# better62/MM-VQA-Healthcare

Measured on AMD Instinct MI355X. Metric: image-question pairs/sec, M3AE-base fine-tune step (fwd+bwd+AdamW) @384px, higher is better.
Workload: dtype bf16

## Files before the change

include/m3ae_hip.h:

```cpp
#ifndef M3AE_HIP_H
#define M3AE_HIP_H

#include <stdint.h>

#ifdef __cplusplus
extern "C" {
#endif

#define M3AE_ABI_VERSION 4

enum { M3AE_F32 = 0, M3AE_BF16 = 1 };
enum { M3AE_ACT_NONE = 0, M3AE_ACT_GELU = 1, M3AE_ACT_QUICKGELU = 2, M3AE_ACT_TANH = 3, M3AE_ACT_RELU = 4,
       M3AE_ACT_MULAUX = 5  };
enum { M3AE_ERR_ARG = -1, M3AE_ERR_UNSUPPORTED = -2, M3AE_ERR_ALIGN = -3, M3AE_ERR_WORKSPACE = -4 };

int m3ae_abi_version(void);
void m3ae_desc_sizes(int64_t out3[3]);
const char* m3ae_last_gemm_path(void);

typedef struct {
    int64_t M, N, K;
    int64_t batch1, batch2;
    const void* A; int64_t a_sm, a_sk, a_sb1, a_sb2;
    const void* B; int64_t b_sk, b_sn, b_sb1, b_sb2;
// ... 44 lines not shown
    float* delta;
    float* d_pos_bias;
    float dropout_p;
    uint64_t dropout_seed;
    const void* dropout_salt;
    int32_t launch_flags;
} m3ae_attn_desc;
enum { M3AE_ATTN_LEGACY_KERNELS = 1,
       M3AE_ATTN_F32_X3 = 2    };
int64_t m3ae_attn_workspace_bytes(const m3ae_attn_desc* d, int backward);
int m3ae_attn_fwd(const m3ae_attn_desc* d, void* stream);
int m3ae_attn_bwd(const m3ae_attn_desc* d, void* stream);
int m3ae_attn_fwd_rows(const m3ae_attn_desc* d, int64_t row_base, int64_t row_step, void* stream);
int m3ae_attn_bwd_rows(const m3ae_attn_desc* d, int64_t row_base, int64_t row_step, void* stream);
int m3ae_attn_probs(const m3ae_attn_desc* d, float* probs, int64_t p_sb, int64_t p_sh, int64_t p_sq, void* stream);

typedef struct {
    int32_t dir;
    int64_t B, Lq, Lk, D, H;
    const void* x;
    const void* y;
    const float* key_mask;
    const void *wq, *wq_t, *wkv, *wkv_t, *wo, *wo_t;
    const float *bq, *bkv, *bo, *ln_g, *ln_b;
    float ln_eps;
    float dropout_p;
    uint64_t seed_attn, seed_hidden;
    void* proj;
    void* prime;
    float* colbias;
// ... 147 lines not shown
```

mm-vqa-healthcare_amd/m3ae_amd/_lib.py:

```python
import ctypes as C
import os

_PKG = os.path.dirname(os.path.abspath(__file__))
DIAGNOSTIC = os.environ.get("M3AE_DIAGNOSTIC_LIB", "") == "1"
LIB_PATH = os.path.join(_PKG, "lib_diag" if DIAGNOSTIC else "lib", "libm3ae_hip.so")

F32, BF16 = 0, 1
ACT_NONE, ACT_GELU, ACT_QUICKGELU, ACT_TANH, ACT_RELU, ACT_MULAUX = 0, 1, 2, 3, 4, 5

vp, i64, i32, f32 = C.c_void_p, C.c_int64, C.c_int32, C.c_float


class GemmDesc(C.Structure):
    _fields_ = [
        ("M", i64), ("N", i64), ("K", i64), ("batch1", i64), ("batch2", i64),
        ("A", vp), ("a_sm", i64), ("a_sk", i64), ("a_sb1", i64), ("a_sb2", i64),
        ("B", vp), ("b_sk", i64), ("b_sn", i64), ("b_sb1", i64), ("b_sb2", i64),
        ("C", vp), ("c_sm", i64), ("c_sn", i64), ("c_sb1", i64), ("c_sb2", i64),
        ("dtype_a", i32), ("dtype_b", i32), ("dtype_c", i32),
        ("alpha", f32), ("accumulate", i32), ("bias", vp), ("act", i32), ("preact", vp), ("residual", vp),
        ("dact_aux", vp), ("dact", i32), ("force_generic", i32), ("a_rowsum", vp),
        ("dropout_p", f32), ("dropout_seed", C.c_uint64), ("preact_grad", i32), ("launch_flags", i32), ("dropout_salt", vp),
    ]

# ... 13 lines not shown


class XattnDesc(C.Structure):
    _fields_ = [
        ("dir", i32), ("B", i64), ("Lq", i64), ("Lk", i64), ("D", i64), ("H", i64),
        ("x", vp), ("y", vp), ("key_mask", vp),
        ("wq", vp), ("wq_t", vp), ("wkv", vp), ("wkv_t", vp), ("wo", vp), ("wo_t", vp),
        ("bq", vp), ("bkv", vp), ("bo", vp), ("ln_g", vp), ("ln_b", vp),
        ("ln_eps", f32), ("dropout_p", f32), ("seed_attn", C.c_uint64), ("seed_hidden", C.c_uint64),
        ("proj", vp), ("prime", vp), ("colbias", vp), ("probs", vp), ("probs_drop", vp), ("rowsum", vp),
        ("zctx", vp), ("ctx", vp), ("s", vp), ("out", vp), ("mean", vp), ("rstd", vp),
        ("d_out", vp), ("dx", vp), ("dy", vp),
        ("g_wq", vp), ("g_wkv", vp), ("g_wo", vp), ("g_bq", vp), ("g_bkv", vp), ("g_bo", vp), ("g_ln_g", vp), ("g_ln_b", vp),
        ("ws_ds", vp), ("ws_dsd", vp), ("ws_dscores", vp), ("ws_dprime", vp), ("ws_dproj", vp), ("ws_dz", vp), ("ws_dctx", vp),
        ("ws_vec", vp), ("ws_ln", vp), ("launch_flags", i32), ("dropout_salt", vp),
    ]


GEMM_NO_PERSISTENT, GEMM_F32_X3, GEMM_DETERMINISTIC = 1, 2, 4
DET_COLSUM, DET_EMBED_BWD, DET_BCE, DET_XENT, DET_MIM = 0, 1, 2, 3, 4
ATTN_LEGACY_KERNELS, ATTN_F32_X3 = 1, 2
XATTN_NO_PERSISTENT, XATTN_LEGACY_CHAIN = 1, 2
ABI_VERSION = 4


_SIGS = {
    "m3ae_abi_version": (C.c_int, []),
    "m3ae_desc_sizes": (None, [C.POINTER(i64)]),
    "m3ae_last_gemm_path": (C.c_char_p, []),
    "m3ae_gemm": (C.c_int, [C.POINTER(GemmDesc), vp]),
# ... 48 lines not shown
    "m3ae_xent_det": (C.c_int, [vp, vp, vp, vp, i64, i64, i64, f32, C.c_int, vp, i64, vp]),
    "m3ae_mim_loss_fwd_det": (C.c_int, [vp, vp, vp, vp, vp, i64, i64, i64, C.c_int, vp, i64, vp]),
    "m3ae_image_resample_workspace_bytes": (i64, [i64, i64]),
    "m3ae_image_resample_u8": (C.c_int, [vp, i64, vp, vp, i64, i64, i64, vp, i64, vp, vp, C.POINTER(C.c_float), C.POINTER(C.c_float), vp]),
    "m3ae_gemm_rows": (C.c_int, [C.POINTER(GemmDesc), i64, i64, vp]),
    "m3ae_attn_fwd_rows": (C.c_int, [C.POINTER(AttnDesc), i64, i64, vp]),
    "m3ae_attn_bwd_rows": (C.c_int, [C.POINTER(AttnDesc), i64, i64, vp]),
    "m3ae_layernorm_bwd_drop_rows": (C.c_int, [vp, vp, vp, vp, vp, vp, vp, vp, f32, C.c_uint64, vp, vp, vp, vp, i64, i64, C.c_int, i64, i64, vp]),
    "m3ae_dropout_rows": (C.c_int, [vp, vp, vp, i64, i64, f32, C.c_uint64, vp, C.c_int, i64, i64, vp]),
    "m3ae_beam_topk_workspace_bytes": (i64, [i64, i64, i64, i64]),
    "m3ae_beam_topk": (C.c_int, [vp, i64, vp, i64, i64, i64, i64, vp, i64, vp, vp, vp]),
    "m3ae_beam_step": (C.c_int, [vp, vp, vp, vp, vp, vp, vp, vp, vp, vp, vp, vp, vp, vp, i64, i64, i64, i64, i64, i64, i64, C.c_double, vp]),
    "m3ae_beam_finalize": (C.c_int, [vp, vp, vp, vp, vp, vp, vp, vp, vp, i64, i64, i64, i64, i64, i64, C.c_double, vp]),
    "m3ae_expand_samples": (C.c_int, [vp, vp, vp, i64, i64, i64, C.c_int, vp]),
    "m3ae_segment_sum_rows": (C.c_int, [vp, vp, vp, vp, i64, i64, i64, C.c_int, vp]),
}

EXPORTS = tuple(_SIGS)
_lib = None


class M3AEHipError(RuntimeError):
    pass


def lib():
    global _lib
    if _lib is None:
        if not os.path.exists(LIB_PATH):
            raise M3AEHipError(f"{LIB_PATH} is missing: build it with `python -m m3ae_amd.build` "
# ... 1 lines not shown
        import torch
        if DIAGNOSTIC:
            import warnings
            warnings.warn(f"m3ae_amd: loading the DIAGNOSTIC library {LIB_PATH} (timing-only builds may compute wrong results)")
        l = C.CDLL(LIB_PATH)
        for name, (res, args) in _SIGS.items():
            fn = getattr(l, name)
            fn.restype, fn.argtypes = res, args
        if l.m3ae_abi_version() != ABI_VERSION:
            raise M3AEHipError(f"ABI version mismatch: library {l.m3ae_abi_version()}, binding {ABI_VERSION}")
        sizes = (i64 * 3)()
        l.m3ae_desc_sizes(sizes)
        mine = (C.sizeof(GemmDesc), C.sizeof(AttnDesc), C.sizeof(XattnDesc))
        if tuple(sizes) != mine:
            raise M3AEHipError(f"descriptor layout mismatch: library {tuple(sizes)}, binding {mine}")
        _lib = l
    return _lib


def check(rc, what):
    if rc != 0:
        kind = {-1: "invalid argument", -2: "unsupported shape/dtype", -3: "misaligned", -4: "workspace too small"}.get(
            rc, f"hipError_t {rc}" if rc > 0 else f"error {rc}")
        raise M3AEHipError(f"{what} failed: {kind}")
```

mm-vqa-healthcare_amd/m3ae_amd/ops.py:

```python
import contextlib
import ctypes as C
import functools
import math
import os
import threading

import torch

from . import _lib
from ._lib import (ACT_GELU, ACT_MULAUX, ACT_NONE, ACT_QUICKGELU, ACT_RELU, ACT_TANH, BF16, F32, AttnDesc, GemmDesc, XattnDesc,
                   check)

grad_ready_hook = None
SAVE_DACT = os.environ.get("M3AE_SAVE_DACT", "1") != "0"
NT_NO_PERSISTENT = os.environ.get("M3AE_NT_NO_PERSISTENT", "0") == "1"
GEMM_NT_VARIANT, GEMM_TN_VARIANT, GEMM_COL_GROUP = int(os.environ.get("M3AE_GEMM_NT_VARIANT", -1)), int(os.environ.get("M3AE_GEMM_TN_VARIANT", -1)), int(os.environ.get("M3AE_GEMM_COL_GROUP", 0))


ATTN_LEGACY = os.environ.get("M3AE_ATTN_LEGACY", "0") == "1"
GEMM_ST_POLICY = int(os.environ.get("M3AE_GEMM_ST_POLICY", 0))


def _gemm_flags():
    return ((1 if NT_NO_PERSISTENT else 0) | (((GEMM_NT_VARIANT + 1) & 0xF) << 8) | (((GEMM_TN_VARIANT + 1) & 0xF) << 12)
            | ((GEMM_COL_GROUP & 0xF) << 16) | ((GEMM_ST_POLICY & 0x3) << 20))
PROFILE = None
# ... 635 lines not shown
    d = _attn_desc(B, heads, Lq, Lk, Dh, q, k, v, o, key_mask, pos_bias, scale, causal, lse, lse.shape[-1], _dt(q))
    delta = torch.empty_like(lse) if q.dtype == torch.bfloat16 else torch.zeros_like(lse)
    d.d_o, d.dq, d.dk, d.dv, d.delta = do.data_ptr(), dq.data_ptr(), dk.data_ptr(), dv.data_ptr(), delta.data_ptr()
    d.d_pos_bias = d_pos_bias.data_ptr() if d_pos_bias is not None else None
    _set_dropout(d, dropout)
    ws = _attn_ws(d, True, q.device)
    e0 = _prof_begin()
    if rows is not None:
        check(_lib.lib().m3ae_attn_bwd_rows(C.byref(d), rows[0], rows[1], _stream()), "m3ae_attn_bwd_rows")
    else:
        check(_lib.lib().m3ae_attn_bwd(C.byref(d), _stream()), "m3ae_attn_bwd")
    _prof_end(e0, "attn_bwd", (B, heads, Lq, Lk, Dh))
    del ws, delta


def attn_probs(q, k, lse, heads, key_mask=None, scale=None, dropout=None):
    _need_cuda(q)
    B, Lq, D = q.shape
    Lk = k.shape[1]
    Dh = D // heads
    if q.dtype == torch.bfloat16 and Dh != 64:
        return attn_probs(q.float(), k.float(), None, heads, key_mask, scale, dropout)
    scale = (1.0 / math.sqrt(Dh)) if scale is None else scale
    out = torch.empty((B, heads, Lq, Lk), dtype=torch.float32, device=q.device)
    lse_stride = lse.shape[-1] if lse is not None else 0
    d = _attn_desc(B, heads, Lq, Lk, Dh, q, k, k, q, key_mask, None, scale, False, lse, lse_stride, _dt(q))
    _set_dropout(d, dropout)
    e0 = _prof_begin()
    check(_lib.lib().m3ae_attn_probs(C.byref(d), C.c_void_p(out.data_ptr()), out.stride(0), out.stride(1), out.stride(2),
                                     _stream()), "m3ae_attn_probs")
# ... 48 lines not shown


def cross_attention(q, kv, key_mask, heads, dropout=None):
    return CrossAttnFn.apply(q, kv, key_mask, heads, dropout)


def _bdata(b):
    return None if b is None else (b.data if hasattr(b, "members") else b.detach())


XATTN = os.environ.get("M3AE_XATTN", "auto")
XATTN_TRAIN = os.environ.get("M3AE_XATTN_TRAIN", "auto")
XATTN_TRAIN_MIN_BATCH = int(os.environ.get("M3AE_XATTN_TRAIN_MIN_BATCH", 96))
XATTN_LEGACY_CHAIN = False
CLS_ONLY = os.environ.get("M3AE_CLS_ONLY", "1") != "0"


def _xattn_desc(h2, B, L, other2, Lo, mask, P, pdrop, seeds):
    D = h2.shape[1]
    d = XattnDesc()
    d.dir = 0 if L <= Lo else 1
    d.B, d.Lq, d.Lk, d.D, d.H = B, L, Lo, D, P.heads
    d.x, d.y = h2.data_ptr(), other2.data_ptr()
    d.key_mask = mask.data_ptr() if mask is not None else None
    wq, wkv, wo = P.w_q, P.w_kv, P.w_o
    d.wq, d.wkv, d.wo = compute_weight(wq).data_ptr(), compute_weight(wkv).data_ptr(), compute_weight(wo).data_ptr()
    d.wq_t, d.wkv_t, d.wo_t = wq.m3ae_t.data_ptr(), wkv.m3ae_t.data_ptr(), wo.m3ae_t.data_ptr()
    d.bq, d.bkv, d.bo = _bdata(P.b_q).data_ptr(), _bdata(P.b_kv).data_ptr(), _bdata(P.b_o).data_ptr()
    d.ln_g, d.ln_b, d.ln_eps = P.ln.weight.data_ptr(), P.ln.bias.data_ptr(), P.ln.eps
    if pdrop > 0:
# ... 234 lines not shown


class _ProjRows:

    def __init__(self, w_param, b_param, r0=None, r1=None):
        self.w_param, self.b_param, self.sl = w_param, b_param, slice(r0, r1)

    @property
    def w(self):
        return compute_weight(self.w_param)[self.sl]

    @property
    def b(self):
        return _bdata(self.b_param)[self.sl]

    def dgrad(self, dy, residual=None):
        M, n = dy.shape
        wt = getattr(self.w_param, "m3ae_t", None)
        if wt is not None:
            b = wt[:, self.sl]
            b_sk, b_sn, K = 1, wt.stride(0), wt.shape[0]
        else:
            b = self.w
            b_sk, b_sn, K = b.stride(0), 1, b.shape[1]
        out = torch.empty((M, K), dtype=dy.dtype, device=dy.device)
        gemm(dy, dy.stride(0), 1, b, b_sk, b_sn, out, K, M, K, n, residual=residual)
        return out

    def wgrad(self, dy, x2, ldx):
        want_b = self.b_param is not None and self.b_param.requires_grad
        if not self.w_param.requires_grad:
            if want_b:
                colsum(dy, _grad_buf(self.b_param)[self.sl], True)
            return
        g = _grad_buf(self.w_param)[self.sl]
        M, n = dy.shape
        gemm(dy, 1, dy.stride(0), x2, ldx, 1, g, g.stride(0), n, g.shape[1], M, accumulate=True,
             a_rowsum=_grad_buf(self.b_param)[self.sl] if want_b else None)


def _live_proj(P, D):
    if hasattr(P, "w_qkv"):
        return _ProjRows(P.w_qkv, P.b_qkv, 0, D), _ProjRows(P.w_qkv, P.b_qkv, D, 3 * D)
    return _ProjRows(P.w_q, P.b_q), _ProjRows(P.w_kv, P.b_kv)


def _attn_sub_fwd_live(hq, src2, B, Ls, Lfull, mask, P, pdrop=0.0):
    D = hq.shape[1]
    da, dh = dropout_pair(pdrop), dropout_pair(pdrop)
    pq, pkv = _live_proj(P, D)
    kv, _ = mm_nt(src2, src2.shape[1], B * Ls, pkv.w, bias=pkv.b)
    q, _ = mm_nt(hq, D, B, pq.w, bias=pq.b)
    n = q.shape[1]
    kv3 = kv.view(B, Ls, 2 * n)
    o, lse = attn_forward(q.view(B, 1, n), kv3[..., :n], kv3[..., n:], P.heads, mask, dropout=da, rows=(0, Lfull))
    s, _ = mm_nt(o.view(B, n), n, B, compute_weight(P.w_o), bias=_bdata(P.b_o), residual=hq, dropout=dh, rows=(0, Lfull))
    y, mean, rstd = ln_fwd_raw(s, P.ln)
    return y, (hq, src2, q, kv, o, lse, s, mean, rstd, mask, da, dh, Ls, Lfull)


def _attn_sub_bwd_live(dy, saved, B, P, need_dsrc=True):
    hq, src2, q, kv, o, lse, s, mean, rstd, mask, da, dh, Ls, Lfull = saved
    D, n = hq.shape[1], q.shape[1]
    ds, dsd = _post_ln_bwd(dy, s, P.ln, mean, rstd, dh, rows=(0, Lfull))
    mm_wgrad(dsd, o.view(B, n), n, P.w_o, P.b_o)
    dctx = mm_dgrad(dsd, P.w_o)
    dq, dkv = torch.empty_like(q), torch.empty_like(kv)
    kv3, dkv3 = kv.view(B, Ls, 2 * n), dkv.view(B, Ls, 2 * n)
    attn_backward(q.view(B, 1, n), kv3[..., :n], kv3[..., n:], o, lse, dctx.view(o.shape), dq.view(B, 1, n), dkv3[..., :n],
                  dkv3[..., n:], P.heads, mask, dropout=da, rows=(0, Lfull))
    pq, pkv = _live_proj(P, D)
    pq.wgrad(dq, hq, D)
    pkv.wgrad(dkv, src2, src2.shape[1])
    for prm in {id(p): p for p in (pq.w_param, pq.b_param, pkv.w_param, pkv.b_param)}.values():
        if prm.requires_grad:
            _done(prm)
    if pq.w_param is pkv.w_param:
        dh = pkv.dgrad(dkv)
        dqkv0 = torch.cat([dq, dkv3[:, 0]], dim=1)
        dh.view(B, Ls, D)[:, 0] = mm_dgrad(dqkv0, pq.w_param, residual=ds)
        return None, dh
    dhq = pq.dgrad(dq, residual=ds)
    return dhq, (pkv.dgrad(dkv) if need_dsrc else None)


class BertCrossLayerFn(Function):

    @staticmethod
    def forward(ctx, h, other, mask_self, mask_other, P, *anchors):
        B, L, D = h.shape
        Lo = other.shape[1]
        h2 = h.contiguous().view(B * L, D)
        other2 = other.contiguous().view(B * Lo, other.shape[2])
        pd = getattr(P, "pdrop", 0.0)
        ctx.live = bool(getattr(P, "cls_only", False))
        if ctx.live:
            hq = h2.view(B, L, D)[:, 0].contiguous()
            a, s1 = _attn_sub_fwd_live(hq, h2, B, L, L, mask_self, P.attn, pd)
# ... 710 lines not shown
```

Measured before the change: 1431.

## Absorb K/V projections into query for CLS-only attention sublayers

For CLS-only cross and self attention layers, the query is folded through the key weights (qt = q·Wk per head), and attention runs directly over the raw source hidden states. The value projection is applied after the weighted sum, through new fused HIP forward and backward kernels with split-K reduction. This avoids computing and storing the full B·Ls×2D K/V projection and its dgrad/wgrad GEMMs for every source token, replacing them with per-head GEMMs on tiny matrices. It adds complex custom MFMA kernels, is gated on shape, mask and dtype conditions, and uses fp32 side buffers.

```diff
diff --git a/include/m3ae_hip.h b/include/m3ae_hip.h
--- a/include/m3ae_hip.h
+++ b/include/m3ae_hip.h
@@ -82,6 +82,33 @@
 int m3ae_attn_fwd_rows(const m3ae_attn_desc* d, int64_t row_base, int64_t row_step, void* stream);
 int m3ae_attn_bwd_rows(const m3ae_attn_desc* d, int64_t row_base, int64_t row_step, void* stream);
 int m3ae_attn_probs(const m3ae_attn_desc* d, float* probs, int64_t p_sb, int64_t p_sh, int64_t p_sq, void* stream);
+
+typedef struct {
+    int64_t B, H, Ls, Ds;
+    const void* qt;
+    const void* src; int64_t src_sb, src_sl;
+    float scale;
+    float dropout_p;
+    uint64_t dropout_seed;
+    const void* dropout_salt;
+    int64_t row_base, row_step;
+    int32_t splits;
+    const float* bv;
+    void* z; float* lse; float* sp; void* vb;
+    float* z32;
+    void* workspace; int64_t workspace_bytes;
+    const void* dz;
+    const void* dctx;
+    void* dqt;
+    void* dsrc; int64_t dsrc_sb, dsrc_sl;
+    const void* dsrc_add0;
+    float* dbv;
+    float* dsrc_row0;
+} m3ae_cls_attn_desc;
+int64_t m3ae_cls_attn_desc_size(void);
+int64_t m3ae_cls_attn_workspace_bytes(const m3ae_cls_attn_desc* d, int backward);
+int m3ae_cls_attn_fwd(const m3ae_cls_attn_desc* d, void* stream);
+int m3ae_cls_attn_bwd(const m3ae_cls_attn_desc* d, void* stream);
 
 typedef struct {
     int32_t dir;
diff --git a/mm-vqa-healthcare_amd/csrc/cls_attn.hip b/mm-vqa-healthcare_amd/csrc/cls_attn.hip
--- /dev/null
+++ b/mm-vqa-healthcare_amd/csrc/cls_attn.hip
@@ -0,0 +1,554 @@
+#include "launch.h"
+
+namespace {
+
+constexpr float LOG2E = 1.4426950408889634f;
+constexpr int DS = 768, HEADS = 12, HP = 16, HW = 64;
+constexpr int NW = 4, DW = DS / NW;
+constexpr int NDT = DW / 32, NKS = DW / 16, NSUB = DW / 64;
+constexpr int VRS = 192;
+constexpr int SUBIMG = 32 * VRS, WIMG = NSUB * SUBIMG;
+constexpr int SROW = 36;
+constexpr int SPART = HP * SROW;
+constexpr int KT = 32;
+constexpr int PART = 3 * HP + HEADS * DS;
+
+DEVINL f32x16 mfma32(s16x8 a, s16x8 b, f32x16 c) {
+    return __builtin_amdgcn_mfma_f32_32x32x16_bf16(__builtin_bit_cast(bf16x8_t, a), __builtin_bit_cast(bf16x8_t, b), c, 0, 0, 0);
+}
+DEVINL int crow(int reg, int h) { return (reg & 3) + 8 * (reg >> 2) + 4 * h; }
+DEVINL s16x8 pack_acc(const f32x16& p, int s) {
+    u32x4 w;
+#pragma unroll
+    for (int i = 0; i < 4; ++i) w[i] = pack2bf(p[8 * s + 2 * i], p[8 * s + 2 * i + 1]);
+    return __builtin_bit_cast(s16x8, w);
+}
+DEVINL s16x8 pack8(const float* x) {
+    u32x4 w;
+#pragma unroll
+    for (int i = 0; i < 4; ++i) w[i] = pack2bf(x[2 * i], x[2 * i + 1]);
+    return __builtin_bit_cast(s16x8, w);
+}
+DEVINL s16x8 lds_row_frag(const char* tile, int r, int ks, int h) { return *(const s16x8*)(tile + r * VRS + 32 * ks + 16 * h); }
+DEVINL s16x8 tr_frag(const char* tile, int dt, int s, int lane) {
+    const int h = lane >> 5, gg = (lane >> 4) & 1, i16 = lane & 15, qq = i16 >> 2, p = i16 & 3;
+    const int row = 16 * s + 4 * h + qq;
+    const int dcol = 32 * dt + 16 * gg + 4 * p;
+    typedef __attribute__((address_space(3))) s16x4 lds_s16x4;
+    const s16x4 lo = __builtin_amdgcn_ds_read_tr16_b64_v4i16((lds_s16x4*)(tile + row * VRS + dcol * 2));
+    const s16x4 hi = __builtin_amdgcn_ds_read_tr16_b64_v4i16((lds_s16x4*)(tile + (row + 8) * VRS + dcol * 2));
+    return (s16x8){lo[0], lo[1], lo[2], lo[3], hi[0], hi[1], hi[2], hi[3]};
+}
+DEVINL f32x16 zero16() {
+    f32x16 z;
+#pragma unroll
+    for (int i = 0; i < 16; ++i) z[i] = 0.f;
+    return z;
+}
+DEVINL s16x8 zero_frag() { return (s16x8){0, 0, 0, 0, 0, 0, 0, 0}; }
+DEVINL float fast_exp2(float x) { return __builtin_amdgcn_exp2f(x); }
+DEVINL void wg_barrier() {
+    asm volatile("s_waitcnt lgkmcnt(0)" ::: "memory");
+    __builtin_amdgcn_s_barrier();
+    asm volatile("" ::: "memory");
+}
+
+struct ClsArgs {
+    const bf16_t* qt;
+    const bf16_t* src; int64_t src_sb, src_sl;
+    float scale, scale_log2;
+    int64_t B, Ls;
+    int nsplit, tps;
+    DropState drop;
+    float* part;
+    const bf16_t* dz;
+    const float* lse; const float* dsp; const float* delta;
+    bf16_t* dsrc; int64_t dsrc_sb, dsrc_sl;
+    const bf16_t* add0;
+    float* row0;
+};
+
+struct Slice { s16x8 v[4 * NSUB]; };
+DEVINL Slice slice_load(const bf16_t* base, int64_t sl, int64_t key0, int64_t k_end, int lane) {
+    Slice s;
+#pragma unroll
+    for (int i = 0; i < 4 * NSUB; ++i) {
+        const int c = (i & 3) * 64 + lane;
+        int64_t row = key0 + (c >> 3);
+        row = row < k_end ? row : k_end - 1;
+        s.v[i] = *(const s16x8*)(base + row * sl + (i >> 2) * 64 + (c & 7) * 8);
+    }
+    return s;
+}
+DEVINL void slice_store(char* img, const Slice& s, int lane) {
+#pragma unroll
+    for (int i = 0; i < 4 * NSUB; ++i) {
+        const int c = (i & 3) * 64 + lane;
+        *(s16x8*)(img + (i >> 2) * SUBIMG + (c >> 3) * VRS + (c & 7) * 16) = s.v[i];
+    }
+    asm volatile("s_waitcnt lgkmcnt(0)" ::: "memory");
+}
+DEVINL void part_store(float* tab, const f32x16& s, int r, int h) {
+    if (r < HP) {
+#pragma unroll
+        for (int g = 0; g < 4; ++g) *(f32x4*)(tab + r * SROW + 8 * g + 4 * h) = (f32x4){s[4 * g], s[4 * g + 1], s[4 * g + 2], s[4 * g + 3]};
+    }
+}
+DEVINL f32x16 part_sum_heads(const float* tab0, int r, int h) {
+    f32x16 s;
+#pragma unroll
+    for (int w = 0; w < NW; ++w)
+#pragma unroll
+        for (int g = 0; g < 4; ++g) {
+            const f32x4 v = *(const f32x4*)(tab0 + w * SPART + (r & (HP - 1)) * SROW + 8 * g + 4 * h);
+#pragma unroll
+            for (int i = 0; i < 4; ++i) s[4 * g + i] = w ? s[4 * g + i] + v[i] : v[i];
+        }
+    return s;
+}
+DEVINL void part_sum_keys(const float* tab0, int r, int h, float* out) {
+#pragma unroll
+    for (int j = 0; j < 8; ++j) {
+        float s = 0.f;
+#pragma unroll
+        for (int w = 0; w < NW; ++w) {
+            const float v = tab0[w * SPART + (8 * h + j) * SROW + r];
+            s = w ? s + v : v;
+        }
+        out[j] = s;
+    }
+}
+DEVINL void keep4(const DropState& d, uint64_t drow, int64_t key4, float* kf) {
+    kf[0] = kf[1] = kf[2] = kf[3] = 1.f;
+    drop_apply4(d, drow + (uint64_t)key4, kf);
+}
+
+DEVINL void split_range(const ClsArgs& a, int split, int64_t& k_begin, int64_t& k_end) {
+    k_begin = (int64_t)split * a.tps * KT;
+    k_end = k_begin + (int64_t)a.tps * KT;
+    k_end = k_end < a.Ls ? k_end : a.Ls;
+}
+DEVINL uint64_t mask_row(const ClsArgs& a, int64_t b, int head) {
+    return (uint64_t)(drop_row(a.drop, b * HEADS + head) * drop_ld(a.Ls));
+}
+
+constexpr int FWD_LDS = NW * WIMG + 2 * NW * SPART * 4;
+
+template <bool DROP>
+__global__ __launch_bounds__(256, 1) void cls_attn_fwd_kernel(ClsArgs a) {
+    extern __shared__ __attribute__((aligned(16))) char lds[];
+    if (DROP) drop_resolve(a.drop);
+    const int t = threadIdx.x, lane = t & 63;
+    const int wave = __builtin_amdgcn_readfirstlane(t >> 6);
+    const int r = lane & 31, h = lane >> 5;
+    const int split = blockIdx.x;
+    const int64_t b = blockIdx.y;
+    int64_t k_begin, k_end;
+    split_range(a, split, k_begin, k_end);
+    const int nt = (int)((k_end - k_begin + KT - 1) / KT);
+    char* img = lds + wave * WIMG;
+    float* tabs = (float*)(lds + NW * WIMG);
+    const int dbase = wave * DW;
+    const int head = r < HEADS ? r : HEADS - 1;
+
+    s16x8 qf[NKS];
+    {
+        const bf16_t* qp = a.qt + (b * HEADS + head) * DS + dbase + 8 * h;
+#pragma unroll
+        for (int ks = 0; ks < NKS; ++ks) qf[ks] = r < HEADS ? *(const s16x8*)(qp + 16 * ks) : zero_frag();
+    }
+    const uint64_t drow = DROP ? mask_row(a, b, head) : 0;
+    const bf16_t* sbase = a.src + b * a.src_sb + dbase;
+
+    f32x16 acc[NDT];
+#pragma unroll
+    for (int n = 0; n < NDT; ++n) acc[n] = zero16();
+    float m = -1e30f, l = 0.f, sp = 0.f;
+
+    Slice nxt = slice_load(sbase, a.src_sl, k_begin, k_end, lane);
+    for (int kt = 0; kt < nt; ++kt) {
+        const int64_t key0 = k_begin + (int64_t)kt * KT;
+        slice_store(img, nxt, lane);
+        if (kt + 1 < nt) nxt = slice_load(sbase, a.src_sl, key0 + KT, k_end, lane);
+
+        f32x16 s = zero16();
+#pragma unroll
+        for (int ks = 0; ks < NKS; ++ks) s = mfma32(lds_row_frag(img + (ks >> 2) * SUBIMG, r, ks & 3, h), qf[ks], s);
+        float* tab = tabs + (kt & 1) * NW * SPART;
+        part_store(tab + wave * SPART, s, r, h);
+        wg_barrier();
+        s = part_sum_heads(tab, r, h);
+
+        float tmax = -1e30f;
+#pragma unroll
+        for (int reg = 0; reg < 16; ++reg) {
+            float x = s[reg] * a.scale_log2;
+            x = key0 + crow(reg, h) < k_end ? x : -INFINITY;
+            s[reg] = x;
+            tmax = fmaxf(tmax, x);
+        }
+        tmax = fmaxf(tmax, __shfl_xor(tmax, 32, 64));
+        if (__any(tmax > m)) {
+            const float mnew = fmaxf(m, tmax);
+            const float alpha = fast_exp2(m - mnew);
+            m = mnew;
+            l *= alpha; sp *= alpha;
+#pragma unroll
+            for (int n = 0; n < NDT; ++n)
+#pragma unroll
+                for (int reg = 0; reg < 16; ++reg) acc[n][reg] *= alpha;
+        }
+#pragma unroll
+        for (int reg = 0; reg < 16; ++reg) {
+            const float p = fast_exp2(s[reg] - m);
+            s[reg] = p;
+            l += p;
+        }
+        if (DROP) {
+#pragma unroll
+            for (int g = 0; g < 4; ++g) {
+                float x4[4] = {s[4 * g], s[4 * g + 1], s[4 * g + 2], s[4 * g + 3]};
+                drop_apply4(a.drop, drow + (uint64_t)(key0 + 8 * g + 4 * h), x4);
+#pragma unroll
+                for (int i = 0; i < 4; ++i) s[4 * g + i] = x4[i];
+            }
+        }
+#pragma unroll
+        for (int reg = 0; reg < 16; ++reg) sp += s[reg];
+#pragma unroll
+        for (int ss = 0; ss < 2; ++ss) {
+            const s16x8 pb = pack_acc(s, ss);
+#pragma unroll
+            for (int n = 0; n < NDT; ++n)
+                acc[n] = mfma32(tr_frag(img + (n >> 1) * SUBIMG, n & 1, ss, lane), pb, acc[n]);
+        }
+    }
+    l += __shfl_xor(l, 32, 64);
+    sp += __shfl_xor(sp, 32, 64);
+    if (r < HEADS) {
+        float* part = a.part + (b * a.nsplit + split) * PART;
+        if (wave == 0 && h == 0) { part[r] = m; part[HP + r] = l; part[2 * HP + r] = sp; }
+        float* zp = part + 3 * HP + r * DS + dbase + 4 * h;
+#pragma unroll
+        for (int n = 0; n < NDT; ++n)
+#pragma unroll
+            for (int g = 0; g < 4; ++g)
+                *(f32x4*)(zp + 32 * n + 8 * g) = (f32x4){acc[n][4 * g], acc[n][4 * g + 1], acc[n][4 * g + 2], acc[n][4 * g + 3]};
+    }
+}
+
+__global__ __launch_bounds__(DS / 4) void cls_attn_fwd_fold_kernel(const float* __restrict__ part, int nsplit, bf16_t* __restrict__ z,
+                                                                  float* __restrict__ lse, float* __restrict__ sp,
+                                                                  const float* __restrict__ bv, bf16_t* __restrict__ vb,
+                                                                  float* __restrict__ z32) {
+    const int64_t b = blockIdx.x / HEADS;
+    const int head = blockIdx.x % HEADS, t = threadIdx.x;
+    const float* p0 = part + b * nsplit * PART;
+    float M = -1e30f;
+    for (int s = 0; s < nsplit; ++s) M = fmaxf(M, p0[s * PART + head]);
+    float L = 0.f, SP = 0.f;
+    f32x4 acc = {0.f, 0.f, 0.f, 0.f};
+    for (int s = 0; s < nsplit; ++s) {
+        const float* p = p0 + s * PART;
+        const float w = fast_exp2(p[head] - M);
+        L += w * p[HP + head];
+        SP += w * p[2 * HP + head];
+        const f32x4 v = *(const f32x4*)(p + 3 * HP + head * DS + 4 * t);
+        acc += v * w;
+    }
+    const float inv = 1.0f / L;
+    u32x2 o;
+    o[0] = pack2bf(acc[0] * inv, acc[1] * inv);
+    o[1] = pack2bf(acc[2] * inv, acc[3] * inv);
+    *(u32x2*)(z + (b * HEADS + head) * DS + 4 * t) = o;
+    if (z32) *(f32x4*)(z32 + (b * HEADS + head) * DS + 4 * t) = acc * inv;
+    if (t == 0) { lse[b * HEADS + head] = M + log2f(L); sp[b * HEADS + head] = SP * inv; }
+    if (vb && t < HW) vb[b * (HEADS * HW) + head * HW + t] = f2bf(SP * inv * bv[head * HW + t]);
+}
+
+__global__ __launch_bounds__(256) void cls_attn_delta_kernel(const bf16_t* __restrict__ dz, const bf16_t* __restrict__ z,
+                                                             const float* __restrict__ z32, const float* __restrict__ sp, const float* __restrict__ bv,
+                                                             const bf16_t* __restrict__ dctx, float* __restrict__ dsp,
+                                                             float* __restrict__ delta, int64_t BH) {
+    const int lane = threadIdx.x & 63;
+    const int64_t bh = (int64_t)blockIdx.x * 4 + (threadIdx.x >> 6);
+    if (bh >= BH) return;
+    const int head = (int)(bh % HEADS);
+    float d = 0.f;
+    for (int i = lane; i < DS; i += 64) d = fmaf(bf2f(dz[bh * DS + i]), z32 ? z32[bh * DS + i] : bf2f(z[bh * DS + i]), d);
+    d = wave_sum(d);
+    float e = bv ? bv[head * HW + lane] * bf2f(dctx[bh * HW + lane]) : 0.f;
+    e = wave_sum(e);
+    if (lane == 0) { dsp[bh] = e; delta[bh] = fmaf(e, sp[bh], d); }
+}
+constexpr int DBV_PARTS = 16;
+__global__ __launch_bounds__(DBV_PARTS * HW) void cls_attn_dbv_kernel(const float* __restrict__ sp, const bf16_t* __restrict__ dctx,
+                                                                      float* __restrict__ dbv, int64_t B) {
+    __shared__ float red[DBV_PARTS][HW];
+    const int head = blockIdx.x, e = threadIdx.x & (HW - 1), part = threadIdx.x / HW;
+    float s = 0.f;
+    for (int64_t b = part; b < B; b += DBV_PARTS) s = fmaf(sp[b * HEADS + head], bf2f(dctx[b * (HEADS * HW) + head * HW + e]), s);
+    red[part][e] = s;
+    __syncthreads();
+    if (part == 0) {
+        float t = red[0][e];
+#pragma unroll
+        for (int p = 1; p < DBV_PARTS; ++p) t += red[p][e];
+        dbv[head * HW + e] += t;
+    }
+}
+
+constexpr int BWD_LDS = NW * WIMG + 2 * 2 * NW * SPART * 4;
+
+template <bool DROP>
+__global__ __launch_bounds__(256, 1) void cls_attn_bwd_kernel(ClsArgs a) {
+    extern __shared__ __attribute__((aligned(16))) char lds[];
+    if (DROP) drop_resolve(a.drop);
+    const int t = threadIdx.x, lane = t & 63;
+    const int wave = __builtin_amdgcn_readfirstlane(t >> 6);
+    const int r = lane & 31, h = lane >> 5;
+    const int split = blockIdx.x;
+    const int64_t b = blockIdx.y;
+    int64_t k_begin, k_end;
+    split_range(a, split, k_begin, k_end);
+    const int nt = (int)((k_end - k_begin + KT - 1) / KT);
+    char* img = lds + wave * WIMG;
+    float* tabs = (float*)(lds + NW * WIMG);
+    const int dbase = wave * DW;
+    const int head = r < HEADS ? r : HEADS - 1;
+
+    s16x8 qf[NKS], zf[NKS];
+    {
+        const int64_t o = (b * HEADS + head) * DS + dbase + 8 * h;
+#pragma unroll
+        for (int ks = 0; ks < NKS; ++ks) {
+            qf[ks] = r < HEADS ? *(const s16x8*)(a.qt + o + 16 * ks) : zero_frag();
+            zf[ks] = r < HEADS ? *(const s16x8*)(a.dz + o + 16 * ks) : zero_frag();
+        }
+    }
+    s16x8 qT[NDT], zT[NDT];
+#pragma unroll
+    for (int n = 0; n < NDT; ++n)
+#pragma unroll
+        for (int j = 0; j < 8; ++j) {
+            const int hd = 8 * h + j;
+            const int64_t o = (b * HEADS + (hd < HEADS ? hd : 0)) * DS + dbase + 32 * n + r;
+            qT[n][j] = hd < HEADS ? (short)a.qt[o] : (short)0;
+            zT[n][j] = hd < HEADS ? (short)a.dz[o] : (short)0;
+        }
+    const float lse_r = a.lse[b * HEADS + head], dsp_r = a.dsp[b * HEADS + head], delta_r = a.delta[b * HEADS + head];
+    const uint64_t drow_r = DROP ? mask_row(a, b, head) : 0;
+    float lse_k[8], dsp_k[8], delta_k[8];
+    uint64_t drow_k[8];
+#pragma unroll
+    for (int j = 0; j < 8; ++j) {
+        const int hd = 8 * h + j < HEADS ? 8 * h + j : HEADS - 1;
+        lse_k[j] = a.lse[b * HEADS + hd]; dsp_k[j] = a.dsp[b * HEADS + hd]; delta_k[j] = a.delta[b * HEADS + hd];
+        drow_k[j] = DROP ? mask_row(a, b, hd) : 0;
+    }
+    const bf16_t* sbase = a.src + b * a.src_sb + dbase;
+    const bool want_dsrc = a.dsrc != nullptr;
+    bf16_t* dbase_p = a.dsrc + (want_dsrc ? b * a.dsrc_sb + dbase : 0);
+
+    f32x16 dq[NDT];
+#pragma unroll
+    for (int n = 0; n < NDT; ++n) dq[n] = zero16();
+
+    Slice nxt = slice_load(sbase, a.src_sl, k_begin, k_end, lane);
+    for (int kt = 0; kt < nt; ++kt) {
+        const int64_t key0 = k_begin + (int64_t)kt * KT;
+        slice_store(img, nxt, lane);
+        if (kt + 1 < nt) nxt = slice_load(sbase, a.src_sl, key0 + KT, k_end, lane);
+
+        f32x16 s = zero16(), dp = zero16();
+#pragma unroll
+        for (int ks = 0; ks < NKS; ++ks) {
+            const s16x8 xf = lds_row_frag(img + (ks >> 2) * SUBIMG, r, ks & 3, h);
+            s = mfma32(xf, qf[ks], s);
+            dp = mfma32(xf, zf[ks], dp);
+        }
+        float* tab = tabs + (kt & 1) * 2 * NW * SPART;
+        part_store(tab + wave * SPART, s, r, h);
+        part_store(tab + (NW + wave) * SPART, dp, r, h);
+        wg_barrier();
+
+        s = part_sum_heads(tab, r, h);
+        dp = part_sum_heads(tab + NW * SPART, r, h);
+#pragma unroll
+        for (int g = 0; g < 4; ++g) {
+            float kf[4] = {1.f, 1.f, 1.f, 1.f};
+            if (DROP) keep4(a.drop, drow_r, key0 + 8 * g + 4 * h, kf);
+#pragma unroll
+            for (int i = 0; i < 4; ++i) {
+                const int reg = 4 * g + i;
+                const float p = key0 + crow(reg, h) < k_end ? fast_exp2(fmaf(s[reg], a.scale_log2, -lse_r)) : 0.f;
+                s[reg] = a.scale * p * (kf[i] * (dp[reg] + dsp_r) - delta_r);
+            }
+        }
+#pragma unroll
+        for (int ss = 0; ss < 2; ++ss) {
+            const s16x8 pb = pack_acc(s, ss);
+#pragma unroll
+            for (int n = 0; n < NDT; ++n) dq[n] = mfma32(tr_frag(img + (n >> 1) * SUBIMG, n & 1, ss, lane), pb, dq[n]);
+        }
+
+        if (!want_dsrc) continue;
+        float sk[8], dk[8], cds[8], pt[8];
+        part_sum_keys(tab, r, h, sk);
+        part_sum_keys(tab + NW * SPART, r, h, dk);
+        const int64_t key = key0 + r;
+#pragma unroll
+        for (int j = 0; j < 8; ++j) {
+            const float p = (key < k_end && 8 * h + j < HEADS) ? fast_exp2(fmaf(sk[j], a.scale_log2, -lse_k[j])) : 0.f;
+            float kf = 1.f;
+            if (DROP) kf = drop_keep(a.drop, drow_k[j] + (uint64_t)key) ? a.drop.inv_keep : 0.f;
+            pt[j] = p * kf;
+            cds[j] = a.scale * p * (kf * (dk[j] + dsp_k[j]) - delta_k[j]);
+        }
+        const s16x8 bds = pack8(cds), bpt = pack8(pt);
+#pragma unroll
+        for (int n = 0; n < NDT; ++n) {
+            f32x16 dx = mfma32(qT[n], bds, zero16());
+            dx = mfma32(zT[n], bpt, dx);
+            if (key < k_end) {
+                bf16_t* rowp = dbase_p + key * a.dsrc_sl + 32 * n + 4 * h;
+                const bf16_t* addp = (a.add0 && key == 0) ? a.add0 + b * DS + dbase + 32 * n + 4 * h : nullptr;
+                float* row0p = (a.row0 && key == 0) ? a.row0 + b * DS + dbase + 32 * n + 4 * h : nullptr;
+#pragma unroll
+                for (int g = 0; g < 4; ++g) {
+                    float v[4] = {dx[4 * g], dx[4 * g + 1], dx[4 * g + 2], dx[4 * g + 3]};
+                    if (addp) {
+#pragma unroll
+                        for (int i = 0; i < 4; ++i) v[i] += bf2f(addp[8 * g + i]);
+                    }
+                    if (row0p) *(f32x4*)(row0p + 8 * g) = (f32x4){v[0], v[1], v[2], v[3]};
+                    u32x2 w;
+                    w[0] = pack2bf(v[0], v[1]);
+                    w[1] = pack2bf(v[2], v[3]);
+                    *(u32x2*)(rowp + 8 * g) = w;
+                }
+            }
+        }
+    }
+    if (r < HEADS) {
+        float* qp = a.part + ((b * a.nsplit + split) * HEADS + r) * DS + dbase + 4 * h;
+#pragma unroll
+        for (int n = 0; n < NDT; ++n)
+#pragma unroll
+            for (int g = 0; g < 4; ++g)
+                *(f32x4*)(qp + 32 * n + 8 * g) = (f32x4){dq[n][4 * g], dq[n][4 * g + 1], dq[n][4 * g + 2], dq[n][4 * g + 3]};
+    }
+}
+
+__global__ __launch_bounds__(DS / 4) void cls_attn_bwd_fold_kernel(const float* __restrict__ part, int nsplit, bf16_t* __restrict__ dqt) {
+    const int64_t b = blockIdx.x / HEADS;
+    const int head = blockIdx.x % HEADS, t = threadIdx.x;
+    f32x4 acc = {0.f, 0.f, 0.f, 0.f};
+    for (int s = 0; s < nsplit; ++s) acc += *(const f32x4*)(part + ((b * nsplit + s) * HEADS + head) * DS + 4 * t);
+    u32x2 o;
+    o[0] = pack2bf(acc[0], acc[1]);
+    o[1] = pack2bf(acc[2], acc[3]);
+    *(u32x2*)(dqt + (b * HEADS + head) * DS + 4 * t) = o;
+}
+
+void split_plan(const m3ae_cls_attn_desc& d, int& nsplit, int& tps) {
+    const int64_t ntiles = cdiv(d.Ls, KT);
+    int64_t want = d.splits > 0 ? d.splits : cdiv(device_cus(), d.B);
+    want = want < 1 ? 1 : (want > ntiles ? ntiles : want);
+    tps = (int)cdiv(ntiles, want);
+    nsplit = (int)cdiv(ntiles, tps);
+}
+int64_t align16(int64_t n) { return (n + 15) & ~(int64_t)15; }
+
+bool al(const void* p, uintptr_t n) { return (((uintptr_t)p) & (n - 1)) == 0; }
+
+int check_common(const m3ae_cls_attn_desc& d) {
+    if (d.B <= 0 || d.H <= 0 || d.Ls <= 0 || d.Ds <= 0 || !d.qt || !d.src || !d.lse || !d.sp || !d.z) return M3AE_ERR_ARG;
+    if (d.splits < 0) return M3AE_ERR_ARG;
+    if (d.B > INT64_MAX / d.H || !drop_rows_ok(DropRows{d.row_base, d.row_step}, d.B * d.H, d.Ls)) return M3AE_ERR_ARG;
+    if (d.dropout_p < 0.f || d.dropout_p >= 1.f) return M3AE_ERR_ARG;
+    if (d.Ds != DS || d.H != HEADS || d.B > 65535) return M3AE_ERR_UNSUPPORTED;
+    if (!al(d.qt, 16) || !al(d.src, 16) || !al(d.z, 16) || !al(d.z32, 16) || d.src_sl % 8 || d.src_sb % 8 || d.src_sl < DS)
+        return M3AE_ERR_UNSUPPORTED;
+    if (!al(d.lse, 4) || !al(d.sp, 4) || !al(d.bv, 4) || !al(d.vb, 2)) return M3AE_ERR_UNSUPPORTED;
+    return 0;
+}
+ClsArgs to_args(const m3ae_cls_attn_desc& d, int nsplit, int tps) {
+    ClsArgs a{};
+    a.qt = (const bf16_t*)d.qt;
+    a.src = (const bf16_t*)d.src; a.src_sb = d.src_sb; a.src_sl = d.src_sl;
+    a.scale = d.scale; a.scale_log2 = d.scale * LOG2E;
+    a.B = d.B; a.Ls = d.Ls;
+    a.nsplit = nsplit; a.tps = tps;
+    a.drop = make_drop(d.dropout_p, d.dropout_seed, d.dropout_salt, DropRows{d.row_base, d.row_step});
+    return a;
+}
+
+}
+
+extern "C" int64_t m3ae_cls_attn_desc_size(void) { return (int64_t)sizeof(m3ae_cls_attn_desc); }
+
+extern "C" int64_t m3ae_cls_attn_workspace_bytes(const m3ae_cls_attn_desc* d, int backward) {
+    if (!d || d->B <= 0 || d->Ls <= 0 || d->splits < 0) return 0;
+    int nsplit, tps;
+    split_plan(*d, nsplit, tps);
+    if (backward) return align16(2 * d->B * HEADS * 4) + d->B * nsplit * HEADS * DS * 4;
+    return d->B * nsplit * (int64_t)PART * 4;
+}
+
+extern "C" int m3ae_cls_attn_fwd(const m3ae_cls_attn_desc* dp, void* stream) {
+    if (!dp) return M3AE_ERR_ARG;
+    const m3ae_cls_attn_desc& d = *dp;
+    if (int rc = check_common(d)) return rc;
+    if ((d.bv == nullptr) != (d.vb == nullptr)) return M3AE_ERR_ARG;
+    if (!d.workspace || (((uintptr_t)d.workspace) & 15) || d.workspace_bytes < m3ae_cls_attn_workspace_bytes(dp, 0)) return M3AE_ERR_WORKSPACE;
+    int nsplit, tps;
+    split_plan(d, nsplit, tps);
+    ClsArgs a = to_args(d, nsplit, tps);
+    a.part = (float*)d.workspace;
+    hipStream_t s = (hipStream_t)stream;
+    const dim3 grid((unsigned)nsplit, (unsigned)d.B);
+    int rc = d.dropout_p > 0.f ? launch_dyn<cls_attn_fwd_kernel<true>>(grid, dim3(256), FWD_LDS, s, a)
+                               : launch_dyn<cls_attn_fwd_kernel<false>>(grid, dim3(256), FWD_LDS, s, a);
+    if (rc) return rc;
+    hipLaunchKernelGGL(cls_attn_fwd_fold_kernel, dim3((unsigned)(d.B * HEADS)), dim3(DS / 4), 0, s, a.part, nsplit, (bf16_t*)d.z, d.lse, d.sp,
+                       d.bv, (bf16_t*)d.vb, d.z32);
+    return hip_launch_status();
+}
+
+extern "C" int m3ae_cls_attn_bwd(const m3ae_cls_attn_desc* dp, void* stream) {
+    if (!dp) return M3AE_ERR_ARG;
+    const m3ae_cls_attn_desc& d = *dp;
+    if (int rc = check_common(d)) return rc;
+    if (!d.dz || !d.dqt) return M3AE_ERR_ARG;
+    if (!d.dsrc && (d.dsrc_add0 || d.dsrc_row0)) return M3AE_ERR_ARG;
+    if ((d.bv != nullptr) != (d.dctx != nullptr) || (d.dbv && !d.bv)) return M3AE_ERR_ARG;
+    if (!al(d.dz, 16) || !al(d.dqt, 16) || !al(d.dsrc, 16) || !al(d.dsrc_add0, 16) || !al(d.dsrc_row0, 16) || !al(d.dctx, 2) || !al(d.dbv, 4))
+        return M3AE_ERR_UNSUPPORTED;
+    if (d.dsrc && (d.dsrc_sl % 8 || d.dsrc_sb % 8 || d.dsrc_sl < DS)) return M3AE_ERR_UNSUPPORTED;
+    if (!d.workspace || (((uintptr_t)d.workspace) & 15) || d.workspace_bytes < m3ae_cls_attn_workspace_bytes(dp, 1)) return M3AE_ERR_WORKSPACE;
+    int nsplit, tps;
+    split_plan(d, nsplit, tps);
+    ClsArgs a = to_args(d, nsplit, tps);
+    float* dsp = (float*)d.workspace;
+    float* delta = dsp + d.B * HEADS;
+    a.part = (float*)((char*)d.workspace + align16(2 * d.B * HEADS * 4));
+    a.dz = (const bf16_t*)d.dz;
+    a.lse = d.lse; a.dsp = dsp; a.delta = delta;
+    a.dsrc = (bf16_t*)d.dsrc; a.dsrc_sb = d.dsrc_sb; a.dsrc_sl = d.dsrc_sl;
+    a.add0 = (const bf16_t*)d.dsrc_add0;
+    a.row0 = d.dsrc_row0;
+    hipStream_t s = (hipStream_t)stream;
+    const int64_t BH = d.B * HEADS;
+    hipLaunchKernelGGL(cls_attn_delta_kernel, dim3((unsigned)cdiv(BH, 4)), dim3(256), 0, s, a.dz, (const bf16_t*)d.z, d.z32, d.sp, d.bv,
+                       (const bf16_t*)d.dctx, dsp, delta, BH);
+    if (d.dbv)
+        hipLaunchKernelGGL(cls_attn_dbv_kernel, dim3(HEADS), dim3(DBV_PARTS * HW), 0, s, d.sp, (const bf16_t*)d.dctx, d.dbv, d.B);
+    if (int rc = hip_launch_status()) return rc;
+    const dim3 grid((unsigned)nsplit, (unsigned)d.B);
+    int rc = d.dropout_p > 0.f ? launch_dyn<cls_attn_bwd_kernel<true>>(grid, dim3(256), BWD_LDS, s, a)
+                               : launch_dyn<cls_attn_bwd_kernel<false>>(grid, dim3(256), BWD_LDS, s, a);
+    if (rc) return rc;
+    hipLaunchKernelGGL(cls_attn_bwd_fold_kernel, dim3((unsigned)BH), dim3(DS / 4), 0, s, a.part, nsplit, (bf16_t*)d.dqt);
+    return hip_launch_status();
+}
diff --git a/mm-vqa-healthcare_amd/m3ae_amd/_lib.py b/mm-vqa-healthcare_amd/m3ae_amd/_lib.py
--- a/mm-vqa-healthcare_amd/m3ae_amd/_lib.py
+++ b/mm-vqa-healthcare_amd/m3ae_amd/_lib.py
@@ -51,6 +51,18 @@
         ("g_wq", vp), ("g_wkv", vp), ("g_wo", vp), ("g_bq", vp), ("g_bkv", vp), ("g_bo", vp), ("g_ln_g", vp), ("g_ln_b", vp),
         ("ws_ds", vp), ("ws_dsd", vp), ("ws_dscores", vp), ("ws_dprime", vp), ("ws_dproj", vp), ("ws_dz", vp), ("ws_dctx", vp),
         ("ws_vec", vp), ("ws_ln", vp), ("launch_flags", i32), ("dropout_salt", vp),
+    ]
+
+
+class ClsAttnDesc(C.Structure):
+    _fields_ = [
+        ("B", i64), ("H", i64), ("Ls", i64), ("Ds", i64),
+        ("qt", vp), ("src", vp), ("src_sb", i64), ("src_sl", i64),
+        ("scale", f32), ("dropout_p", f32), ("dropout_seed", C.c_uint64), ("dropout_salt", vp),
+        ("row_base", i64), ("row_step", i64), ("splits", i32), ("bv", vp),
+        ("z", vp), ("lse", vp), ("sp", vp), ("vb", vp), ("z32", vp), ("workspace", vp), ("workspace_bytes", i64),
+        ("dz", vp), ("dctx", vp), ("dqt", vp), ("dsrc", vp), ("dsrc_sb", i64), ("dsrc_sl", i64), ("dsrc_add0", vp), ("dbv", vp),
+        ("dsrc_row0", vp),
     ]
 
 
@@ -129,6 +141,10 @@
     "m3ae_beam_finalize": (C.c_int, [vp, vp, vp, vp, vp, vp, vp, vp, vp, i64, i64, i64, i64, i64, i64, C.c_double, vp]),
     "m3ae_expand_samples": (C.c_int, [vp, vp, vp, i64, i64, i64, C.c_int, vp]),
     "m3ae_segment_sum_rows": (C.c_int, [vp, vp, vp, vp, i64, i64, i64, C.c_int, vp]),
+    "m3ae_cls_attn_desc_size": (i64, []),
+    "m3ae_cls_attn_workspace_bytes": (i64, [C.POINTER(ClsAttnDesc), C.c_int]),
+    "m3ae_cls_attn_fwd": (C.c_int, [C.POINTER(ClsAttnDesc), vp]),
+    "m3ae_cls_attn_bwd": (C.c_int, [C.POINTER(ClsAttnDesc), vp]),
 }
 
 EXPORTS = tuple(_SIGS)
@@ -160,6 +176,8 @@
         mine = (C.sizeof(GemmDesc), C.sizeof(AttnDesc), C.sizeof(XattnDesc))
         if tuple(sizes) != mine:
             raise M3AEHipError(f"descriptor layout mismatch: library {tuple(sizes)}, binding {mine}")
+        if l.m3ae_cls_attn_desc_size() != C.sizeof(ClsAttnDesc):
+            raise M3AEHipError(f"m3ae_cls_attn_desc layout mismatch: library {l.m3ae_cls_attn_desc_size()}, binding {C.sizeof(ClsAttnDesc)}")
         _lib = l
     return _lib
 
diff --git a/mm-vqa-healthcare_amd/m3ae_amd/ops.py b/mm-vqa-healthcare_amd/m3ae_amd/ops.py
--- a/mm-vqa-healthcare_amd/m3ae_amd/ops.py
+++ b/mm-vqa-healthcare_amd/m3ae_amd/ops.py
@@ -8,8 +8,8 @@
 import torch
 
 from . import _lib
-from ._lib import (ACT_GELU, ACT_MULAUX, ACT_NONE, ACT_QUICKGELU, ACT_RELU, ACT_TANH, BF16, F32, AttnDesc, GemmDesc, XattnDesc,
-                   check)
+from ._lib import (ACT_GELU, ACT_MULAUX, ACT_NONE, ACT_QUICKGELU, ACT_RELU, ACT_TANH, BF16, F32, AttnDesc, ClsAttnDesc, GemmDesc,
+                   XattnDesc, check)
 
 grad_ready_hook = None
 SAVE_DACT = os.environ.get("M3AE_SAVE_DACT", "1") != "0"
@@ -675,6 +675,73 @@
     del ws, delta
 
 
+def _cls_attn_desc(qt, src3, scale, dropout, rows, splits):
+    B, H, Ds = qt.shape
+    assert qt.is_contiguous() and src3.stride(2) == 1
+    d = ClsAttnDesc()
+    d.B, d.H, d.Ls, d.Ds = B, H, src3.shape[1], Ds
+    d.qt, d.src, d.src_sb, d.src_sl = qt.data_ptr(), src3.data_ptr(), src3.stride(0), src3.stride(1)
+    d.scale = scale
+    d.row_base, d.row_step = rows if rows is not None else (0, 1)
+    d.splits = splits
+    _set_dropout(d, dropout)
+    return d
+
+
+def _cls_attn_ws(d, backward, device):
+    n = _lib.lib().m3ae_cls_attn_workspace_bytes(C.byref(d), int(backward))
+    ws = torch.empty(max(n, 16), dtype=torch.uint8, device=device)
+    d.workspace, d.workspace_bytes = ws.data_ptr(), n
+    return ws
+
+
+def cls_attn_forward(qt, src3, scale, bv=None, dropout=None, rows=None, splits=0, outs=None, z32=None):
+    _need_cuda(qt)
+    B, H, Ds = qt.shape
+    d = _cls_attn_desc(qt, src3, scale, dropout, rows, splits)
+    if outs is not None:
+        z, lse, sp = outs
+    else:
+        z = torch.empty_like(qt)
+        lse = torch.empty((B, H), dtype=torch.float32, device=qt.device)
+        sp = torch.empty_like(lse)
+    vb = torch.empty((B, bv.numel()), dtype=qt.dtype, device=qt.device) if bv is not None else None
+    d.z, d.lse, d.sp, d.bv, d.vb, d.z32 = z.data_ptr(), lse.data_ptr(), sp.data_ptr(), _p(bv), _p(vb), _p(z32)
+    ws = _cls_attn_ws(d, False, qt.device)
+    e0 = _prof_begin()
+    check(_lib.lib().m3ae_cls_attn_fwd(C.byref(d), _stream()), "m3ae_cls_attn_fwd")
+    _prof_end(e0, "cls_attn_fwd", (B, H, 1, src3.shape[1], Ds))
+    del ws
+    return z, lse, sp, vb
+
+
+def cls_attn_backward(qt, src3, z, lse, sp, dz, scale, bv=None, dctx=None, dbv=None, add0=None, dropout=None, rows=None, splits=0,
+                      outs=None, z32=None, need_dsrc=True, row0=None):
+    B, H, Ds = qt.shape
+    Ls = src3.shape[1]
+    d = _cls_attn_desc(qt, src3, scale, dropout, rows, splits)
+    dqt, dsrc = outs if outs is not None else (None, None)
+    if dqt is None:
+        dqt = torch.empty_like(qt)
+    if not need_dsrc:
+        assert dsrc is None and add0 is None and row0 is None
+    elif dsrc is None:
+        dsrc = torch.empty((B, Ls, Ds), dtype=qt.dtype, device=qt.device)
+    assert dqt.is_contiguous() and (dsrc is None or dsrc.stride(2) == 1)
+    assert dz.is_contiguous() and z.is_contiguous() and (dctx is None or dctx.is_contiguous()) and (add0 is None or add0.is_contiguous())
+    assert row0 is None or (row0.dtype == torch.float32 and row0.is_contiguous() and row0.shape == (B, Ds))
+    d.z, d.lse, d.sp, d.bv, d.z32 = z.data_ptr(), lse.data_ptr(), sp.data_ptr(), _p(bv), _p(z32)
+    d.dz, d.dctx, d.dqt, d.dbv, d.dsrc_add0, d.dsrc_row0 = dz.data_ptr(), _p(dctx), dqt.data_ptr(), _p(dbv), _p(add0), _p(row0)
+    if dsrc is not None:
+        d.dsrc, d.dsrc_sb, d.dsrc_sl = dsrc.data_ptr(), dsrc.stride(0), dsrc.stride(1)
+    ws = _cls_attn_ws(d, True, qt.device)
+    e0 = _prof_begin()
+    check(_lib.lib().m3ae_cls_attn_bwd(C.byref(d), _stream()), "m3ae_cls_attn_bwd")
+    _prof_end(e0, "cls_attn_bwd", (B, H, 1, Ls, Ds))
+    del ws
+    return dqt, dsrc
+
+
 def attn_probs(q, k, lse, heads, key_mask=None, scale=None, dropout=None):
     _need_cuda(q)
     B, Lq, D = q.shape
@@ -753,6 +820,8 @@
 XATTN_TRAIN_MIN_BATCH = int(os.environ.get("M3AE_XATTN_TRAIN_MIN_BATCH", 96))
 XATTN_LEGACY_CHAIN = False
 CLS_ONLY = os.environ.get("M3AE_CLS_ONLY", "1") != "0"
+CLS_ABSORB = os.environ.get("M3AE_CLS_ABSORB", "1") != "0"
+CLS_ABSORB_MIN_ROWS = max(2048, int(os.environ.get("M3AE_CLS_ABSORB_MIN_ROWS", 36928)))
 
 
 def _xattn_desc(h2, B, L, other2, Lo, mask, P, pdrop, seeds):
@@ -1017,7 +1086,7 @@
     def b(self):
         return _bdata(self.b_param)[self.sl]
 
-    def dgrad(self, dy, residual=None):
+    def dgrad(self, dy, residual=None, acc=None):
         M, n = dy.shape
         wt = getattr(self.w_param, "m3ae_t", None)
         if wt is not None:
@@ -1026,6 +1095,10 @@
         else:
             b = self.w
             b_sk, b_sn, K = b.stride(0), 1, b.shape[1]
+        if acc is not None:
+            assert residual is None and acc.shape == (M, K) and acc.is_contiguous()
+            gemm(dy, dy.stride(0), 1, b, b_sk, b_sn, acc, K, M, K, n, accumulate=True)
+            return acc
         out = torch.empty((M, K), dtype=dy.dtype, device=dy.device)
         gemm(dy, dy.stride(0), 1, b, b_sk, b_sn, out, K, M, K, n, residual=residual)
         return out
@@ -1048,10 +1121,32 @@
     return _ProjRows(P.w_q, P.b_q), _ProjRows(P.w_kv, P.b_kv)
 
 
+def _cls_absorb(hq, src2, B, Ls, mask, P):
+    return (CLS_ABSORB and not _DETERMINISTIC and mask is None and hq.dtype == torch.bfloat16 and src2.dtype == torch.bfloat16
+            and B * Ls >= CLS_ABSORB_MIN_ROWS and src2.shape[1] == 768 and hq.shape[1] == 768 and P.heads == 12)
+
+
 def _attn_sub_fwd_live(hq, src2, B, Ls, Lfull, mask, P, pdrop=0.0):
     D = hq.shape[1]
     da, dh = dropout_pair(pdrop), dropout_pair(pdrop)
     pq, pkv = _live_proj(P, D)
+    if _cls_absorb(hq, src2, B, Ls, mask, P):
+        q, _ = mm_nt(hq, D, B, pq.w, bias=pq.b)
+        n, H, Ds = q.shape[1], P.heads, src2.shape[1]
+        wk, wv, dhd = pkv.w[:n], pkv.w[n:], n // H
+        qt = torch.empty((B, H, Ds), dtype=q.dtype, device=q.device)
+        gemm(q, n, 1, wk, wk.stride(0), 1, qt, H * Ds, B, Ds, dhd, batch=(H, 1), a_sb=(dhd, 0), b_sb=(dhd * wk.stride(0), 0),
+             c_sb=(Ds, 0))
+        bv = pkv.b[n:] if pkv.b is not None else None
+        z32 = torch.empty((B, H, Ds), dtype=torch.float32, device=q.device)
+        z, lse, sp, vb = cls_attn_forward(qt, src2.view(B, Ls, Ds), 1.0 / math.sqrt(dhd), bv=bv, dropout=da, rows=(0, Lfull),
+                                          z32=z32)
+        o = torch.empty((B, n), dtype=q.dtype, device=q.device)
+        gemm(z, H * Ds, 1, wv, 1, wv.stride(0), o, n, B, dhd, Ds, batch=(H, 1), a_sb=(Ds, 0), b_sb=(dhd * wv.stride(0), 0),
+             c_sb=(dhd, 0), residual=vb)
+        s, _ = mm_nt(o, n, B, compute_weight(P.w_o), bias=_bdata(P.b_o), residual=hq, dropout=dh, rows=(0, Lfull))
+        y, mean, rstd = ln_fwd_raw(s, P.ln)
+        return y, (hq, src2, q, None, o, lse, s, mean, rstd, mask, da, dh, Ls, Lfull, (qt, z, sp, z32))
     kv, _ = mm_nt(src2, src2.shape[1], B * Ls, pkv.w, bias=pkv.b)
     q, _ = mm_nt(hq, D, B, pq.w, bias=pq.b)
     n = q.shape[1]
@@ -1059,15 +1154,17 @@
     o, lse = attn_forward(q.view(B, 1, n), kv3[..., :n], kv3[..., n:], P.heads, mask, dropout=da, rows=(0, Lfull))
     s, _ = mm_nt(o.view(B, n), n, B, compute_weight(P.w_o), bias=_bdata(P.b_o), residual=hq, dropout=dh, rows=(0, Lfull))
     y, mean, rstd = ln_fwd_raw(s, P.ln)
-    return y, (hq, src2, q, kv, o, lse, s, mean, rstd, mask, da, dh, Ls, Lfull)
+    return y, (hq, src2, q, kv, o, lse, s, mean, rstd, mask, da, dh, Ls, Lfull, None)
 
 
 def _attn_sub_bwd_live(dy, saved, B, P, need_dsrc=True):
-    hq, src2, q, kv, o, lse, s, mean, rstd, mask, da, dh, Ls, Lfull = saved
+    hq, src2, q, kv, o, lse, s, mean, rstd, mask, da, dh, Ls, Lfull, absorbed = saved
     D, n = hq.shape[1], q.shape[1]
     ds, dsd = _post_ln_bwd(dy, s, P.ln, mean, rstd, dh, rows=(0, Lfull))
     mm_wgrad(dsd, o.view(B, n), n, P.w_o, P.b_o)
     dctx = mm_dgrad(dsd, P.w_o)
+    if absorbed is not None:
+        return _attn_sub_bwd_absorbed(dctx, ds, saved, B, P, need_dsrc)
     dq, dkv = torch.empty_like(q), torch.empty_like(kv)
     kv3, dkv3 = kv.view(B, Ls, 2 * n), dkv.view(B, Ls, 2 * n)
     attn_backward(q.view(B, 1, n), kv3[..., :n], kv3[..., n:], o, lse, dctx.view(o.shape), dq.view(B, 1, n), dkv3[..., :n],
@@ -1085,6 +1182,42 @@
         return None, dh
     dhq = pq.dgrad(dq, residual=ds)
     return dhq, (pkv.dgrad(dkv) if need_dsrc else None)
+
+
+def _attn_sub_bwd_absorbed(dctx, ds, saved, B, P, need_dsrc):
+    hq, src2, q, _, o, lse, s, mean, rstd, mask, da, dh, Ls, Lfull, (qt, z, sp, z32) = saved
+    D, n, H, Ds = hq.shape[1], q.shape[1], P.heads, src2.shape[1]
+    dhd = n // H
+    pq, pkv = _live_proj(P, D)
+    wk, wv = pkv.w[:n], pkv.w[n:]
+    dz = torch.empty_like(qt)
+    gemm(dctx, n, 1, wv, wv.stride(0), 1, dz, H * Ds, B, Ds, dhd, batch=(H, 1), a_sb=(dhd, 0), b_sb=(dhd * wv.stride(0), 0),
+         c_sb=(Ds, 0))
+    want_w = pkv.w_param.requires_grad
+    want_b = pkv.b_param is not None and pkv.b_param.requires_grad
+    self_attn = pq.w_param is pkv.w_param
+    row0 = torch.empty((B, Ds), dtype=torch.float32, device=q.device) if self_attn else None
+    dqt, dsrc = cls_attn_backward(qt, src2.view(B, Ls, Ds), z, lse, sp, dz, 1.0 / math.sqrt(dhd),
+                                  bv=pkv.b[n:] if pkv.b is not None else None, dctx=dctx if pkv.b is not None else None,
+                                  dbv=_grad_buf(pkv.b_param)[pkv.sl][n:] if want_b else None, add0=ds if self_attn else None,
+                                  dropout=da, rows=(0, Lfull), z32=z32, need_dsrc=need_dsrc or self_attn, row0=row0)
+    dq = torch.empty_like(q)
+    gemm(dqt, H * Ds, 1, wk, 1, wk.stride(0), dq, n, B, dhd, Ds, batch=(H, 1), a_sb=(Ds, 0), b_sb=(dhd * wk.stride(0), 0),
+         c_sb=(dhd, 0))
+    if want_w:
+        g = _grad_buf(pkv.w_param)[pkv.sl]
+        for dy, x3, gs in ((q, dqt, g[:n]), (dctx, z, g[n:])):
+            gemm(dy, 1, n, x3, H * Ds, 1, gs, gs.stride(0), dhd, Ds, B, accumulate=True, batch=(H, 1), a_sb=(dhd, 0),
+                 b_sb=(Ds, 0), c_sb=(dhd * gs.stride(0), 0))
+    pq.wgrad(dq, hq, D)
+    for prm in {id(p): p for p in (pq.w_param, pq.b_param, pkv.w_param, pkv.b_param)}.values():
+        if prm is not None and prm.requires_grad:
+            _done(prm)
+    if self_attn:
+        dsrc[:, 0] = pq.dgrad(dq, acc=row0)
+        return None, dsrc.view(B * Ls, Ds)
+    dhq = pq.dgrad(dq, residual=ds)
+    return dhq, (dsrc.view(B * Ls, Ds) if dsrc is not None else None)
 
 
 class BertCrossLayerFn(Function):
```

Result: no change. 1444, median of 6 (+0.9%).
